# Rocco9999/2048_Q-Learning

Hardware: AMD Instinct MI355X
Metric: env_steps_per_sec (higher is better)
Workload: dtype u8

## Files before the change

### 2048_q-learning_amd/csrc/q2048_kernels.hip

```cpp
#include <hip/hip_runtime.h>
#include <stddef.h>
#include <stdint.h>

#include <cstdio>
#include <cstdlib>
#include <cstring>
#include <ctime>
#include <condition_variable>
#include <deque>
#include <functional>
#include <map>
#include <mutex>
#include <thread>
#include <type_traits>
#include <vector>

#include "q2048_abi.hpp"
#include "q2048_core5.hpp"

#ifdef Q2048_EXPERIMENTS
#define Q2048_XBITS(flags, shift, mask) (((flags) >> (shift)) & (mask))
#else
#define Q2048_XBITS(flags, shift, mask) 0u
#endif
// ... 190 lines not shown
  }
  return kNoSlot;
}

__global__ __launch_bounds__(kBlock) void k_table_summarise(q2048_slot* table, u64 lines) {
  for (u64 l = (u64)blockIdx.x * kBlock + threadIdx.x; l < lines; l += (u64)gridDim.x * kBlock) {
    q2048_slot* s = table + (l << 2);
    u64 sum = 0ull;
#pragma unroll
    for (int r = 0; r < 4; ++r) {
      const u64 k = s[r].key;
      if (k != 0ull) sum |= summary_fp(mix64(k)) << (16 * r);
    }
#pragma unroll
    for (int r = 0; r < 4; ++r) s[r].reserved = sum;
  }
}
__device__ __forceinline__ int64_t probe_find_summary(const q2048_slot* table, u64 mask, const Geo<4>::Key& key,
                                                      Row& row, bool& created, uint32_t maxp = kRolloutProbe) {
  const u64 hash = key_hash(key);
  const Seq sq = seq_of(hash, mask);
  const u64 fp = summary_fp(hash);
  created = false;
  row = Row{0.f, 0.f, 0.f, 0.f};
  for (uint32_t p = 0, lim = probe_limit(mask, maxp); p < lim; p += 4u) {
    const u64 base = ((sq.line0 + (u64)(p >> 2)) & sq.lmask) << 2;
    const u32x4 v = ld16_agent(&table[base | (u64)sq.off].q[2]);
    const u64 sum = (u64)v.z | ((u64)v.w << 32);
    uint32_t e = 0u, m = 0u;
#pragma unroll
    for (uint32_t r = 0; r < 4u; ++r) {
      const u64 f = (sum >> (16u * r)) & 0xffffull;
      e |= (uint32_t)(f == 0ull) << r;
      m |= (uint32_t)(f == fp) << r;
    }
    uint32_t ev = (((e | m) | ((e | m) << 4)) >> sq.off) & 15u;
    while (ev != 0u) {
      const uint32_t j = (uint32_t)__builtin_ctz(ev), r = (sq.off + j) & 3u;
      const u64 i = base | (u64)r;
      if ((e >> r) & 1u) return ~(int64_t)i;
      const u32x4 h = ld16_agent(&table[i]);
      if (((u64)h.x | ((u64)h.y << 32)) == key.k0) {
        u64 hi = (u64)v.x | ((u64)v.y << 32);
        if (j != 0u) hi = ld_u64(&table[i].q[2]);
        row = Row{bits_f32(h.z), bits_f32(h.w), bits_f32((uint32_t)hi), bits_f32((uint32_t)(hi >> 32))};
        return (int64_t)i;
      }
      ev &= ev - 1u;
    }
  }
  return kNoSlot;
}
template <int KEY_WORDS>
__global__ __launch_bounds__(kBlock) void k_table_summarise_side(const q2048_slot* table, u64 lines, u64* side) {
  for (u64 l = (u64)blockIdx.x * kBlock + threadIdx.x; l < lines; l += (u64)gridDim.x * kBlock) {
    const uint4* s = reinterpret_cast<const uint4*>(table + (l << 2));
    u64 sum = 0ull;
#pragma unroll
    for (int r = 0; r < 4; ++r) {
      const uint4 a = s[2 * r];
      const u64 k = (u64)a.x | ((u64)a.y << 32);
      u64 h = k;
      if constexpr (KEY_WORDS == 2) {
        const uint4 b = s[2 * r + 1];
        h = k ^ (((u64)b.z | ((u64)b.w << 32)) * 0x9E3779B97F4A7C15ull);
      }
      if (k != 0ull) sum |= summary_fp(mix64(h)) << (16 * r);
    }
    side[l] = sum;
  }
}
__device__ __forceinline__ int64_t probe_find_summary(const q2048_slot* table, const u64* side, u64 mask,
                                                      const Geo<5>::Key& key, Row& row, bool& created,
                                                      uint32_t maxp = kRolloutProbe) {
  const u64 hash = key_hash(key);
  const Seq sq = seq_of(hash, mask);
  const u64 fp = summary_fp(hash);
  created = false;
  row = Row{0.f, 0.f, 0.f, 0.f};
  for (uint32_t p = 0, lim = probe_limit(mask, maxp); p < lim; p += 4u) {
    const u64 line = (sq.line0 + (u64)(p >> 2)) & sq.lmask;
    SummaryHits hits = summary_decode(ld_u64(&side[line]), fp, sq.off);
    uint32_t r;
    bool absent;
    while (summary_pop(hits, sq.off, r, absent)) {
      const u64 i = (line << 2) | (u64)r;
      if (absent) return ~(int64_t)i;
      const u32x4 a = ld16_agent(&table[i]);
      if (((u64)a.x | ((u64)a.y << 32)) == key.k0) {
        const u32x4 b = ld16_agent(&table[i].q[2]);
        if (((u64)b.z | ((u64)b.w << 32)) == key.k1) {
          row = Row{bits_f32(a.z), bits_f32(a.w), bits_f32(b.x), bits_f32(b.y)};
          return (int64_t)i;
        }
      }
    }
  }
  return kNoSlot;
}
template <bool SUMMARY, class Key>
__device__ __forceinline__ int64_t probe_find_as(const q2048_slot* table, const u64* side, u64 mask, const Key& key,
                                                 Row& row, bool& created) {
  if constexpr (SUMMARY && sizeof(Key) == sizeof(u64)) return probe_find_summary(table, mask, key, row, created);
  else if constexpr (SUMMARY) return probe_find_summary(table, side, mask, key, row, created);
  else return probe_find(table, mask, key, row, created);
}

template <class Key>
__device__ __forceinline__ int64_t probe_insert(q2048_slot* table, u64 mask, const Key& key, u64 start,
                                                bool& inserted, uint32_t maxp = kRolloutProbe) {
  const Seq sq = seq_of(key_hash(key), mask);
  u64 i = start & mask;
  inserted = false;
  u64 k = 0ull;
  for (uint32_t p = seq_pos(sq, i), lim = probe_limit(mask, maxp); p < lim; i = seq_slot(sq, ++p), k = ld_u64(&table[i].key)) {
    if (k == 0ull) k = atomicCAS(reinterpret_cast<u64*>(&table[i].key), 0ull, key.k0);
    if ((k == 0ull || k == key.k0) && confirm(&table[i], key, k == 0ull, inserted)) return (int64_t)i;
  }
  inserted = false;
  return kNoSlot;
}

struct Claim { u64 ret; u64 at; bool active; };

__device__ __forceinline__ int64_t claim_issue(q2048_slot* table, u64, int64_t slot,
                                               const Geo<4>::Key& key, Claim& c, bool&) {
  c.active = slot < 0 && slot != kNoSlot;
  if (c.active) {
    c.at = (u64)~slot;
    c.ret = atomicCAS(reinterpret_cast<u64*>(&table[c.at].key), 0ull, key.k0);
  }
  return slot;
}
__device__ __forceinline__ int64_t claim_issue(q2048_slot* table, u64 mask, int64_t slot,
                                               const Geo<5>::Key& key, Claim& c, bool& inserted) {
  c.active = false;
  if (slot < 0 && slot != kNoSlot) return probe_insert(table, mask, key, (u64)~slot, inserted);
  return slot;
}
template <class Key>
__device__ __forceinline__ int64_t claim_resolve(q2048_slot* table, u64 mask, const Key& key, Claim& c,
                                                 int64_t slot, bool& inserted) {
  if (!c.active) return slot;
  c.active = false;
  if (c.ret == 0ull) { inserted = true; return (int64_t)c.at; }
  if (c.ret == key.k0) return (int64_t)c.at;
  const Seq sq = seq_of(key_hash(key), mask);
  return probe_insert(table, mask, key, seq_slot(sq, seq_pos(sq, c.at) + 1u), inserted);
}

enum : uint32_t { kTdStorePlain = 0, kTdCas = 1, kTdStoreSc1 = 2, kTdStoreNt = 3, kTdNone = 4,
                  kTdAdd = 6 };
struct TdCounters { uint32_t retries, fallbacks; };
__device__ __forceinline__ float td_update(q2048_slot* slot, int a, float guess, float reward,
                                           float max_next, bool done, double lr, double gamma,
                                           TdCounters& ctrs, uint32_t mode, int max_cas = kMaxCas) {
  unsigned int* addr = reinterpret_cast<unsigned int*>(&slot->q[a]);
  unsigned int expect = f32_bits(guess);
  float nq = td_value(guess, reward, max_next, done, lr, gamma);
  if (mode == kTdStorePlain) { *addr = f32_bits(nq); return nq; }
  if (mode == kTdNone) return nq;
#ifdef Q2048_EXPERIMENTS
  if (mode == kTdStoreSc1) {
    __hip_atomic_store(addr, f32_bits(nq), __ATOMIC_RELAXED, __HIP_MEMORY_SCOPE_AGENT);
    return nq;
  }
  if (mode == kTdStoreNt) { __builtin_nontemporal_store(f32_bits(nq), addr); return nq; }
  if (mode == kTdAdd) { atomicAdd(&slot->q[a], nq - guess); return nq; }
#endif
  for (int it = 0; it < max_cas; ++it) {
    const unsigned int prev = atomicCAS(addr, expect, f32_bits(nq));
    if (prev == expect) return nq;
    ++ctrs.retries;
    expect = prev;
    nq = td_value(bits_f32(expect), reward, max_next, done, lr, gamma);
  }
  ++ctrs.fallbacks;
  *addr = f32_bits(nq);
  return nq;
}
__device__ __forceinline__ void flush_pending(q2048_slot* slot, const Row& q, uint32_t& pend) {
  unsigned int* w = reinterpret_cast<unsigned int*>(slot->q);
  if (pend & 1u) w[0] = f32_bits(q.q0);
  if (pend & 2u) w[1] = f32_bits(q.q1);
  if (pend & 4u) w[2] = f32_bits(q.q2);
  if (pend & 8u) w[3] = f32_bits(q.q3);
  pend = 0u;
}
__device__ __forceinline__ uint32_t td_mode_of(uint32_t flags) {
  const uint32_t x = Q2048_XBITS(flags, 8, 15u);
  return x ? x : ((flags & Q2048_FLAG_TD_CAS) ? kTdCas : kTdStorePlain);
}

__device__ __forceinline__ uint32_t wave_count(bool pred) {
  return (uint32_t)__popcll(__ballot(pred));
}
__device__ __forceinline__ bool wave_leader() {
  const u64 active = __ballot(true);
  return (u64)(threadIdx.x & 63) == (u64)__ffsll((long long)active) - 1ull;
}

struct BlockStats {
  u64 i[Q2048_NSTAT_I];
  double f[Q2048_NSTAT_F];
};
__device__ __forceinline__ void stats_clear(BlockStats& s) {
  if (threadIdx.x < Q2048_NSTAT_I) s.i[threadIdx.x] = 0ull;
  if (threadIdx.x < Q2048_NSTAT_F) s.f[threadIdx.x] = 0.0;
  __syncthreads();
}
__device__ __forceinline__ void stats_flush(BlockStats& s, int64_t* gi, double* gf) {
  __syncthreads();
  if (gi != nullptr && threadIdx.x < Q2048_NSTAT_I && s.i[threadIdx.x] != 0ull)
    atomicAdd(reinterpret_cast<u64*>(gi) + threadIdx.x, s.i[threadIdx.x]);
  if (gf != nullptr && threadIdx.x < Q2048_NSTAT_F && s.f[threadIdx.x] != 0.0)
    atomicAdd(gf + threadIdx.x, s.f[threadIdx.x]);
}
constexpr int kStatStripes = 64;
struct StatStripe { u64 i[Q2048_NSTAT_I]; double f[Q2048_NSTAT_F]; };
__device__ __forceinline__ void stats_flush_striped(BlockStats& s, StatStripe* stripes) {
  __syncthreads();
  if (stripes == nullptr) return;
  StatStripe& mine = stripes[blockIdx.x % kStatStripes];
  if (threadIdx.x < Q2048_NSTAT_I && s.i[threadIdx.x] != 0ull) atomicAdd(&mine.i[threadIdx.x], s.i[threadIdx.x]);
  if (threadIdx.x < Q2048_NSTAT_F && s.f[threadIdx.x] != 0.0) atomicAdd(&mine.f[threadIdx.x], s.f[threadIdx.x]);
}
__global__ __launch_bounds__(64) void k_stats_fold(const StatStripe* stripes, int64_t* gi, double* gf) {
  const int t = (int)threadIdx.x;
  if (t < Q2048_NSTAT_I && gi != nullptr) {
    u64 sum = 0ull;
    for (int k = 0; k < kStatStripes; ++k) sum += stripes[k].i[t];
    if (sum) atomicAdd(reinterpret_cast<u64*>(gi) + t, sum);
  } else if (t >= Q2048_NSTAT_I && t < Q2048_NSTAT_I + Q2048_NSTAT_F && gf != nullptr) {
    double sum = 0.0;
    for (int k = 0; k < kStatStripes; ++k) sum += stripes[k].f[t - Q2048_NSTAT_I];
    if (sum != 0.0) atomicAdd(gf + (t - Q2048_NSTAT_I), sum);
  }
}
__device__ __forceinline__ void wait_vm() { asm volatile("s_waitcnt vmcnt(0)" ::: "memory"); }
__device__ __forceinline__ void stats_flush_acked(BlockStats& s, int64_t* gi, double* gf) {
  __syncthreads();
  if (threadIdx.x < Q2048_NSTAT_I && s.i[threadIdx.x] != 0ull) {
    const u64 old = atomicAdd(reinterpret_cast<u64*>(gi) + threadIdx.x, s.i[threadIdx.x]);
    asm volatile("" :: "v"(old));
  }
  if (threadIdx.x < Q2048_NSTAT_F && s.f[threadIdx.x] != 0.0) {
    const double old = atomicAdd(gf + threadIdx.x, s.f[threadIdx.x]);
    asm volatile("" :: "v"(old));
  }
  wait_vm();
}
__device__ __forceinline__ void stats_mirror(const int64_t* gi, const double* gf, u64* mirror, uint32_t* ticket) {
  __shared__ uint32_t my_ticket;
  __syncthreads();
  if (threadIdx.x == 0)
    my_ticket = __hip_atomic_fetch_add(ticket, 1u, __ATOMIC_RELAXED, __HIP_MEMORY_SCOPE_AGENT);
  __syncthreads();
  if (my_ticket != gridDim.x - 1u) return;
  const int t = (int)threadIdx.x;
  if (t < Q2048_NSTAT_I + Q2048_NSTAT_F) {
    const u64* src = t < Q2048_NSTAT_I ? reinterpret_cast<const u64*>(gi) + t
                                       : reinterpret_cast<const u64*>(gf) + (t - Q2048_NSTAT_I);
    const u64 v = __hip_atomic_load(const_cast<u64*>(src), __ATOMIC_RELAXED, __HIP_MEMORY_SCOPE_AGENT);
    __hip_atomic_store(mirror + t, v, __ATOMIC_RELAXED, __HIP_MEMORY_SCOPE_SYSTEM);
  }
  wait_vm();
  __syncthreads();
  if (t == 0) {
    const uint32_t launches = __hip_atomic_load(ticket + 1, __ATOMIC_RELAXED, __HIP_MEMORY_SCOPE_AGENT) + 1u;
    __hip_atomic_store(ticket + 1, launches, __ATOMIC_RELAXED, __HIP_MEMORY_SCOPE_AGENT);
    __hip_atomic_store(mirror + Q2048_MIRROR_SEQ, (u64)launches, __ATOMIC_RELAXED, __HIP_MEMORY_SCOPE_SYSTEM);
    __hip_atomic_store(ticket, 0u, __ATOMIC_RELAXED, __HIP_MEMORY_SCOPE_AGENT);
  }
}
__device__ __forceinline__ void episode_stats(BlockStats& s, const Aux& a, uint32_t max_l2) {
  atomicAdd(&s.i[Q2048_ST_SCORE], (u64)(int64_t)a.score);
  atomicAdd(&s.i[Q2048_ST_HIST0 + (max_l2 > 22u ? 22u : max_l2)], 1ull);
  const double ret = (double)a.ep_return;
  atomicAdd(&s.f[Q2048_SF_RETURN], ret);
  atomicAdd(&s.f[Q2048_SF_RETURN_SQ], ret * ret);
}

template <int N>
__global__ __launch_bounds__(kBlock) void k_env_init(uint8_t* boards, q2048_aux* aux, int64_t B,
                                                     uint64_t seed, uint64_t env_id0) {
  __shared__ Stage<N> st;
  const int64_t i = (int64_t)blockIdx.x * kBlock + threadIdx.x;
  typename Geo<N>::BoardT b;
  Aux a;
  init_env(b, a, seed, env_id0 + (uint64_t)i);
  store_board(boards, i, B, b, st);
  if (i < B) st_aux(aux, i, a);
}

template <int N>
__global__ __launch_bounds__(kBlock) void k_env_reset(uint8_t* boards, q2048_aux* aux,
                                                      const uint8_t* mask, int64_t B, uint64_t seed,
                                                      uint64_t env_id0, uint32_t flags) {
  __shared__ Stage<N> st;
  const int64_t i = (int64_t)blockIdx.x * kBlock + threadIdx.x;
  const bool mine = i < B && (mask == nullptr || mask[i] != 0);
  if constexpr (N == 4) { if (!mine) return; }
  else { if (__ballot(mine) == 0ull) return; }
  auto b = load_board(boards, i, B, st);
  if (mine) {
    Aux a = ld_aux(aux, i);
    begin_episode(b, a, seed, env_id0 + (uint64_t)i, (flags & Q2048_FLAG_RESET_SHAPING) != 0);
    st_aux(aux, i, a);
  }
  store_board(boards, i, B, b, st);
}

template <int N, int ENV>
__global__ __launch_bounds__(kBlock) void k_env_step(const uint8_t* boards_in, uint8_t* boards, q2048_aux* aux,
                                                     const uint8_t* actions, int64_t B, uint64_t seed,
                                                     uint64_t env_id0, uint32_t ctr, float* reward,
                                                     uint8_t* done, uint8_t* max_l2, int32_t* max_tile,
                                                     uint32_t* status,
                                                     const uint32_t* draw_pos, const uint32_t* draw_val,
                                                     const uint32_t* draw_opos, const uint32_t* draw_oval,
                                                     int draw_stride) {
  __shared__ Stage<N> st;
  const int64_t i = (int64_t)blockIdx.x * kBlock + threadIdx.x;
  auto b = load_board(boards_in, i, B, st);
  if (i < B) {
    const int act = actions[i];
    if (act > 3) {
      atomicOr(status, Q2048_STATUS_BAD_ACTION);
// ... 244 lines not shown
  Row r;
  bool made;
  uint32_t g;
  const int64_t slot = probe_find(table, mask, state_key_as<SYM>(b, salt, status, g), r, made, kMaxProbe);
  if constexpr (SYM) r = row_env(r, g);
  reinterpret_cast<float4*>(q_out)[i] = make_float4(r.q0, r.q1, r.q2, r.q3);
  if (found != nullptr) found[i] = slot >= 0;
}

constexpr int kUpdateBlock = 1024;
template <int N, bool FROZEN>
__global__ __launch_bounds__(kUpdateBlock) void k_q_update(q2048_slot* table, u64 mask, const uint8_t* s,
                                                     const uint8_t* actions, const float* reward,
                                                     const uint8_t* s2, const uint8_t* done, int64_t B,
                                                     double lr, double gamma, uint64_t env_id0,
                                                     uint32_t flags, RowCache<N>* cache, int64_t* stats_i,
                                                     uint32_t* status) {
  __shared__ BlockStats bs;
  __shared__ Stage<N, kUpdateBlock / 64> st;
  stats_clear(bs);
  const int64_t i = (int64_t)blockIdx.x * kUpdateBlock + threadIdx.x;
  const auto b_s = load_board(s, i, B, st);
  const auto b_n = load_board(s2, i, B, st);
  if (i < B) {
    const int act = actions[i];
    const float rew = reward[i];
    const bool is_done = done[i] != 0;
    bool ins_n = false, ins_s = false, dropped = false;
    TdCounters tdc{0u, 0u};
    constexpr bool frozen = FROZEN;
    if (act > 3) {
      atomicOr(status, Q2048_STATUS_BAD_ACTION);
    } else {
      const u64 salt = (flags & Q2048_FLAG_INDEPENDENT) ? lane_salt(env_id0 + (uint64_t)i) : 0ull;
      const auto key_s = state_key(b_s, salt, status);
      const auto key_n = state_key(b_n, salt, status);
      const bool same = key_eq(key_n, key_s);
      Row rs;
      int64_t slot = kNoSlot;
      if (cache == nullptr || !cache_get(cache, i, key_s, cache_tag(table, mask), rs, slot, frozen)) {
        slot = probe_find(table, mask, key_s, rs, ins_s);
        if (slot < 0 && slot != kNoSlot && !frozen) slot = probe_insert(table, mask, key_s, (u64)~slot, ins_s);
      }
      Row rn = rs;
      int64_t slot_n = slot;
      Claim claim{0ull, 0ull, false};
      if (!same) {
        slot_n = probe_find(table, mask, key_n, rn, ins_n);
        if constexpr (!frozen) slot_n = claim_issue(table, mask, slot_n, key_n, claim, ins_n);
      }
      const float max_next = max4(rn.q0, rn.q1, rn.q2, rn.q3);
      if (slot >= 0) {
        const float nq = td_update(&table[slot], act, row_get(rs, act), rew, max_next, is_done,
                                   lr, gamma, tdc, td_mode_of(flags));
        if (same) row_set(rn, act, nq);
      } else {
        dropped = true;
        if (!frozen) atomicOr(status, Q2048_STATUS_TABLE_FULL);
        else if (same)
          row_set(rn, act, td_value(row_get(rs, act), rew, max_next, is_done, lr, gamma));
      }
      bool ins_c = false;
      slot_n = claim_resolve(table, mask, key_n, claim, slot_n, ins_c);
      ins_n = ins_n || ins_c;
      if (cache != nullptr) cache_put(cache, i, key_n, cache_tag(table, mask), rn, slot_n, frozen);
    }
    const uint32_t n_ins = wave_count(ins_n) + wave_count(ins_s), n_drop = wave_count(dropped);
    if (tdc.retries) atomicAdd(&bs.i[Q2048_ST_CAS_RETRY], (u64)tdc.retries);
    if (tdc.fallbacks) atomicAdd(&bs.i[Q2048_ST_CAS_FALLBACK], (u64)tdc.fallbacks);
    if (wave_leader()) {
      if (n_ins) atomicAdd(&bs.i[Q2048_ST_INSERTS], (u64)n_ins);
      if (n_drop) atomicAdd(&bs.i[Q2048_ST_DROPS], (u64)n_drop);
    }
  }
  stats_flush(bs, stats_i, nullptr);
}

#ifdef Q2048_FUSED_MIN_WAVES
#define Q2048_FUSED_WAVES(N) Q2048_FUSED_MIN_WAVES
#else
#define Q2048_FUSED_WAVES(N) ((N) == 4 ? 6 : 5)
#endif
constexpr int kModeLearn = 0, kModeCas = 1, kModeEval = 2, kModeFrozen = 4, kModeSummary = 8;
constexpr int kModeSym = 16;
constexpr int kFusedBlockBig = 512, kFusedBlockSmall = kBlock;
constexpr int64_t kFusedBigBatch = 786432;
#ifdef Q2048_EXPERIMENTS
__device__ unsigned long long* g_timeline;
#define Q2048_STAMP(k) do { if (g_timeline != nullptr && threadIdx.x == 0) {                       \
    g_timeline[(size_t)blockIdx.x * 8 + (k)] = wall_clock64();                                     \
    if ((k) == 0) {                                                                                \
      g_timeline[(size_t)blockIdx.x * 8 + 4] = (unsigned)__builtin_amdgcn_s_getreg((31 << 11) | 4);   \
      g_timeline[(size_t)blockIdx.x * 8 + 5] = (unsigned)__builtin_amdgcn_s_getreg((31 << 11) | 20);  \
    } } } while (0)
#else
#define Q2048_STAMP(k) do { } while (0)
#endif
__device__ const LutImage g_lut_image = Q2048_LUT_IMAGE;
template <int N, int ENV, int MODE, int BLOCK>
__global__ __launch_bounds__(BLOCK, Q2048_FUSED_WAVES(N)) void k_fused_rollout(
    uint8_t* boards, q2048_aux* aux, q2048_slot* table, u64 mask, int64_t B, int steps, double eps,
    double lr, double gamma, uint64_t seed, uint64_t env_id0, uint32_t ctr0, uint32_t flags,
    int64_t* stats_i, double* stats_f, uint32_t* status, q2048_episode* log, int64_t log_cap,
    u64* log_count, void* row_cache, u64* mirror, uint32_t* ticket, const u64* side) {
  RowCache<N>* const cache = static_cast<RowCache<N>*>(row_cache);
  __shared__ BlockStats bs;
  __shared__ Stage<N, BLOCK / 64> st;
  __shared__ LutImage lut_lds;
  static_assert(BLOCK >= kLutImageDoubles, "one double of the image per thread");
  Q2048_STAMP(0);
  if (threadIdx.x < kLutImageDoubles)
    reinterpret_cast<double*>(&lut_lds)[threadIdx.x] = reinterpret_cast<const double*>(&g_lut_image)[threadIdx.x];
  stats_clear(bs);
  const ImageLuts lut{&lut_lds};
  const int64_t i = (int64_t)blockIdx.x * BLOCK + threadIdx.x;
  auto b = load_board(boards, i, B, st);
  if (i < B) {
    const uint64_t id = env_id0 + (uint64_t)i;
    const u64 salt = (flags & Q2048_FLAG_INDEPENDENT) ? lane_salt(id) : 0ull;
    constexpr bool play_only = (ENV & kEnvPlayOnly) != 0;
    constexpr bool no_learn = (MODE & ~kModeSym) == kModeEval;
    constexpr bool sym = (MODE & kModeSym) != 0;
    static_assert(!sym || (N == 4 && !play_only), "symmetry folding: 4x4 learners, evaluators and frozen tables");
    constexpr bool frozen = (MODE & kModeFrozen) != 0;
    constexpr bool summary = (MODE & kModeSummary) != 0;
#ifdef Q2048_EXPERIMENTS
    const uint32_t td_mode = no_learn ? (uint32_t)kTdNone : td_mode_of(flags);
    const bool x_noclaim = ((flags >> 12) & 1u) || play_only || no_learn || frozen, x_noprobe = ((flags >> 13) & 1u) || play_only;
    const bool may_defer = td_mode == kTdStorePlain && !((flags >> 14) & 1u);
    const int max_cas = ((flags >> 16) & 0xffu) ? (int)((flags >> 16) & 0xffu) : kMaxCas;
#else
    constexpr uint32_t td_mode = no_learn ? kTdNone : ((MODE & kModeCas) ? kTdCas : kTdStorePlain);
    constexpr bool x_noclaim = play_only || no_learn || frozen, x_noprobe = play_only;
    constexpr bool may_defer = td_mode == kTdStorePlain;
    constexpr int max_cas = kMaxCas;
#endif
    Aux a = ld_aux(aux, i);
    uint32_t g_s;
    auto key_s = state_key_as<sym>(b, salt, status, g_s);
    Row q{0.f, 0.f, 0.f, 0.f};
    bool made0 = false;
    int64_t slot_s = kNoSlot;
    if (!play_only && (cache == nullptr || !cache_get(cache, i, key_s, cache_tag(table, mask), q, slot_s, frozen)))
      slot_s = probe_find_as<summary>(table, side, mask, key_s, q, made0);
    Claim claim{0ull, 0ull, false};
    uint32_t n_valid = 0, n_explore = 0, n_done = 0, n_insert = wave_count(made0), n_drop = 0;
    uint32_t pend = 0;
    TdCounters tdc{0u, 0u};
    double reward_sum = 0.0;
    const DrawPrep prep_x = draws_prepare(seed, id, kStreamStep);
    const uint64_t eps_t = eps_threshold(eps);

    for (int t = 0; t < steps; ++t) {
      const Draws x = draws_at(prep_x, ctr0 + (uint32_t)t);
      Draws y{0u, 0u, 0u, 0u};
      if constexpr ((ENV & kEnvDqn) != 0) y = draws(seed, id, ctr0 + (uint32_t)t, kStreamOver);
      bool explored;
      Row qe = q;
      if constexpr (sym) qe = row_env(q, g_s);
      const int act_env = eps_greedy_at(eps_t, x.x0, x.x1, qe.q0, qe.q1, qe.q2, qe.q3, explored);
      const StepOut o = env_step_profile<ENV>(b, a, act_env, x.x2, x.x3, y.x0, y.x1, lut);
      const int act = sym ? sym_action(g_s, act_env) : act_env;
      uint32_t g_n;
      const auto key_n = state_key_as<sym>(b, salt, status, g_n);
      const bool same = key_eq(key_n, key_s);
      bool ins_s = false, ins_n = false;
      slot_s = claim_resolve(table, mask, key_s, claim, slot_s, ins_s);
      if (slot_s < 0 && slot_s != kNoSlot && !x_noclaim)
        slot_s = probe_insert(table, mask, key_s, (u64)~slot_s, ins_s);
      Row qn = q;
      int64_t slot_n = slot_s;
      if (!same) {
        if (x_noprobe) { qn = Row{0.f, 0.f, 0.f, 0.f}; slot_n = ~(int64_t)key_home(key_n, mask); }
        else slot_n = probe_find_as<summary>(table, side, mask, key_n, qn, ins_n);
      }
      const float max_next = max4(qn.q0, qn.q1, qn.q2, qn.q3);
      float nq = 0.f;
      const bool updated = slot_s >= 0;
      if (updated) {
        if (same && !o.done && may_defer) {
          nq = td_value(row_get(q, act), o.reward, max_next, false, lr, gamma);
          pend |= 1u << act;
        } else {
          nq = td_update(&table[slot_s], act, row_get(q, act), o.reward, max_next, o.done != 0, lr,
                         gamma, tdc, td_mode, max_cas);
          pend &= ~(1u << act);
          if (pend) flush_pending(&table[slot_s], q, pend);
        }
      } else if (frozen) {
        nq = td_value(row_get(q, act), o.reward, max_next, o.done != 0, lr, gamma);
      }
      if (o.done) {
        if (!same && slot_n < 0 && slot_n != kNoSlot && !x_noclaim)
          probe_insert(table, mask, key_n, (u64)~slot_n, ins_n);
        episode_stats(bs, a, o.max_log2);
        if (log != nullptr) {
          const u64 at = atomicAdd(log_count, 1ull);
          if ((int64_t)at < log_cap) {
            Row ql = q;
            if ((updated || frozen) && !no_learn) row_set(ql, act, nq);
            if constexpr (sym) ql = row_env(ql, g_s);
            q2048_episode rec;
            rec.env_id = id; rec.episode = a.episode; rec.action = (uint8_t)act_env;
            rec.max_log2 = o.max_log2; rec.steps_lo = (uint16_t)(ctr0 + (uint32_t)t);
            rec.reward = o.reward; rec.total_return = a.ep_return; rec.score = a.score;
            rec.q[0] = ql.q0; rec.q[1] = ql.q1; rec.q[2] = ql.q2; rec.q[3] = ql.q3;
            rec.reserved = 0u;
            log[at] = rec;
          }
        }
        begin_episode(b, a, seed, id, (ENV & kEnvResetShaping) != 0);
        key_s = state_key_as<sym>(b, salt, status, g_s);
        bool made = false;
        q = Row{0.f, 0.f, 0.f, 0.f};
        slot_s = play_only ? kNoSlot : probe_find_as<summary>(table, side, mask, key_s, q, made);
        ins_n = ins_n || made;
      } else if (same) {
        if ((updated || frozen) && !no_learn) row_set(q, act, nq);
        else if (!updated) slot_s = kNoSlot;
      } else {
        key_s = key_n; slot_s = slot_n; q = qn; g_s = g_n;
        if (!x_noclaim) {
          bool made = false;
          slot_s = claim_issue(table, mask, slot_s, key_s, claim, made);
          ins_n = ins_n || made;
        }
      }
      n_valid += wave_count(o.valid != 0);
      n_explore += wave_count(explored);
      n_insert += wave_count(ins_s) + wave_count(ins_n);
      n_drop += wave_count(!updated && !play_only && !no_learn);
      n_done += wave_count(o.done != 0);
      reward_sum += (double)o.reward;
      if (t == 0) Q2048_STAMP(1);
    }
    Q2048_STAMP(2);
    if (pend && slot_s >= 0) flush_pending(&table[slot_s], q, pend);
    bool ins_last = false;
    slot_s = claim_resolve(table, mask, key_s, claim, slot_s, ins_last);
    n_insert += wave_count(ins_last);
    st_aux(aux, i, a);
    if (!play_only && cache != nullptr) cache_put(cache, i, key_s, cache_tag(table, mask), q, slot_s, frozen);

    if (n_drop && !frozen) atomicOr(status, Q2048_STATUS_TABLE_FULL);
    if (tdc.retries) atomicAdd(&bs.i[Q2048_ST_CAS_RETRY], (u64)tdc.retries);
    if (tdc.fallbacks) atomicAdd(&bs.i[Q2048_ST_CAS_FALLBACK], (u64)tdc.fallbacks);
    atomicAdd(&bs.f[Q2048_SF_REWARD], reward_sum);
    const uint32_t n_active = wave_count(true);
    if (wave_leader()) {
      atomicAdd(&bs.i[Q2048_ST_STEPS], (u64)n_active * (u64)steps);
      atomicAdd(&bs.i[Q2048_ST_VALID], (u64)n_valid);
      atomicAdd(&bs.i[Q2048_ST_EXPLORE], (u64)n_explore);
      atomicAdd(&bs.i[Q2048_ST_EPISODES], (u64)n_done);
      atomicAdd(&bs.i[Q2048_ST_INSERTS], (u64)n_insert);
      atomicAdd(&bs.i[Q2048_ST_DROPS], (u64)n_drop);
    }
  }
  store_board(boards, i, B, b, st);
  if (mirror == nullptr) {
    stats_flush(bs, stats_i, stats_f);
  } else {
    stats_flush_acked(bs, stats_i, stats_f);
    stats_mirror(stats_i, stats_f, mirror, ticket);
  }
  Q2048_STAMP(3);
}

template <int N, int ENV, bool SYM = false>
__global__ __launch_bounds__(kBlock) void k_play_rollout(
    uint8_t* boards, q2048_aux* aux, const q2048_slot* table, u64 mask, int64_t B, int steps, double eps,
    uint64_t seed, uint64_t env_id0, uint32_t ctr0, uint32_t flags, int64_t* stats_i, double* stats_f,
    uint32_t* status) {
  __shared__ BlockStats bs;
  __shared__ Stage<N> st;
  __shared__ LutImage lut_lds;
  static_assert(kBlock >= kLutImageDoubles, "one double of the image per thread");
  if (threadIdx.x < kLutImageDoubles)
    reinterpret_cast<double*>(&lut_lds)[threadIdx.x] = reinterpret_cast<const double*>(&g_lut_image)[threadIdx.x];
  stats_clear(bs);
  const ImageLuts lut{&lut_lds};
  const int64_t i = (int64_t)blockIdx.x * kBlock + threadIdx.x;
  auto b = load_board(boards, i, B, st);
  if (i < B) {
    const uint64_t id = env_id0 + (uint64_t)i;
    const u64 salt = (flags & Q2048_FLAG_INDEPENDENT) ? lane_salt(id) : 0ull;
    Aux a = ld_aux(aux, i);
    uint32_t n_valid = 0, n_explore = 0, n_done = 0;
    double reward_sum = 0.0;
    const DrawPrep prep_x = draws_prepare(seed, id, kStreamStep);
    const uint64_t eps_t = eps_threshold(eps);
    for (int t = 0; t < steps; ++t) {
      const Draws x = draws_at(prep_x, ctr0 + (uint32_t)t);
      Draws y{0u, 0u, 0u, 0u};
      if constexpr ((ENV & kEnvDqn) != 0) y = draws(seed, id, ctr0 + (uint32_t)t, kStreamOver);
      Row q;
      bool made;
      uint32_t g;
      probe_find(table, mask, state_key_as<SYM>(b, salt, status, g), q, made, kMaxProbe);
      if constexpr (SYM) q = row_env(q, g);
      bool explored;
      const int act = play_action(legal_mask(b), q.q0, q.q1, q.q2, q.q3, eps_t, x.x0, x.x1, explored);
      const StepOut o = env_step_profile<ENV>(b, a, act, x.x2, x.x3, y.x0, y.x1, lut);
      if (o.done) {
        episode_stats(bs, a, o.max_log2);
        begin_episode(b, a, seed, id, (ENV & kEnvResetShaping) != 0);
      }
      n_valid += wave_count(o.valid != 0);
      n_explore += wave_count(explored);
      n_done += wave_count(o.done != 0);
      reward_sum += (double)o.reward;
    }
    st_aux(aux, i, a);
    atomicAdd(&bs.f[Q2048_SF_REWARD], reward_sum);
    const uint32_t n_active = wave_count(true);
    if (wave_leader()) {
      atomicAdd(&bs.i[Q2048_ST_STEPS], (u64)n_active * (u64)steps);
      atomicAdd(&bs.i[Q2048_ST_VALID], (u64)n_valid);
      atomicAdd(&bs.i[Q2048_ST_EXPLORE], (u64)n_explore);
      atomicAdd(&bs.i[Q2048_ST_EPISODES], (u64)n_done);
    }
  }
  store_board(boards, i, B, b, st);
  stats_flush(bs, stats_i, stats_f);
}

constexpr int kDetHashShift = 44, kDetHashBits = 16;
constexpr u64 kDetSlotMask = (1ull << kDetHashShift) - 1ull;
constexpr u64 kDetDrop = 1ull << 62, kDetDone = 1ull << 63;
constexpr uint32_t kNoCarry = 0xffffffffu;
__device__ __forceinline__ Row ld_row(const q2048_slot* s) {
  const u32x4 v = ld16_agent(&s->q[0]);
  return Row{bits_f32(v.x), bits_f32(v.y), bits_f32(v.z), bits_f32(v.w)};
}
template <int N, int ENV, bool VISITS>
__device__ __forceinline__ void det_phase1_body(
    uint8_t* boards, q2048_aux* aux, q2048_slot* table, u64 mask, int64_t B, double eps, double gamma,
    uint64_t seed, uint64_t env_id0, uint32_t ctr, uint32_t flags, u64* group_out, double* target_out,
    uint32_t* carry, int use_carry, StatStripe* stat_stripes, uint32_t* gs0, int n_gs, uint32_t* status,
    RowCache<N>* cache, double lr) {
  __shared__ BlockStats bs;
  __shared__ Stage<N> st;
  stats_clear(bs);
  const int64_t i = (int64_t)blockIdx.x * kBlock + threadIdx.x;
  for (int64_t idx = i; idx < (int64_t)n_gs; idx += (int64_t)gridDim.x * kBlock) gs0[idx] = 0u;
  auto b = load_board(boards, i, B, st);
  if (i < B) {
    const uint64_t id = env_id0 + (uint64_t)i;
    const u64 salt = (flags & Q2048_FLAG_INDEPENDENT) ? lane_salt(id) : 0ull;
    Aux a = ld_aux(aux, i);
    const auto key_s = state_key(b, salt, status);
    const u64 hash_s = key_hash(key_s);
    const Draws x = draws(seed, id, ctr, kStreamStep);
    Draws y{0u, 0u, 0u, 0u};
    if constexpr ((ENV & kEnvDqn) != 0) y = draws(seed, id, ctr, kStreamOver);
    Row q{0.f, 0.f, 0.f, 0.f}, qn;
    bool ins_s = false, ins_n = false, dropped = false;
    const bool frozen = (flags & Q2048_FLAG_NO_NEW_ROWS) != 0u;
    const uint32_t held = use_carry ? carry[i] : kNoCarry;
    constexpr bool visits = VISITS;
    int64_t slot_s;
    if (held != kNoCarry) {
      slot_s = (int64_t)held;
      if (!(draw_uniform(x.x0) < eps)) q = ld_row(&table[slot_s]);
    } else {
      slot_s = probe_find(table, mask, key_s, q, ins_s);
      if (slot_s < 0 && slot_s != kNoSlot && !frozen) slot_s = probe_insert(table, mask, key_s, (u64)~slot_s, ins_s);
      if (slot_s < 0) { dropped = true; if (!frozen || slot_s == kNoSlot) atomicOr(status, Q2048_STATUS_TABLE_FULL); }
      if constexpr (visits) {
        if (slot_s < 0) {
          Row v;
          int64_t at;
          if (cache_get(cache, i, key_s, cache_tag(table, mask), v, at, true) && at == kNoSlot) q = v;
        }
      }
    }
    bool explored;
    const int act = eps_greedy(eps, x.x0, x.x1, q.q0, q.q1, q.q2, q.q3, explored);
    const StepOut o = env_step_profile<ENV>(b, a, act, x.x2, x.x3, y.x0, y.x1);
// ... 3656 lines not shown
```

Baseline: 22.59 billion.

## Skip next-state probe on terminal steps and defer missed-slot inserts via claims

On terminal transitions the TD update now uses a specialized terminal value that ignores max_next, so the next-state probe is skipped and only the fresh episode's start state is probed. Missing-key inserts that used to be synchronous probe_insert calls are now issued as asynchronous claims, at the top of the next iteration or on the terminal path, and resolved later. This aims to cut hash-table probes and serialized atomic inserts per step. It restructures the claim/resolve ordering and the terminal bookkeeping, which risks subtle changes in insert counts or in which slot gets updated.

```diff
diff --git a/2048_q-learning_amd/csrc/q2048_kernels.hip b/2048_q-learning_amd/csrc/q2048_kernels.hip
--- a/2048_q-learning_amd/csrc/q2048_kernels.hip
+++ b/2048_q-learning_amd/csrc/q2048_kernels.hip
@@ -366,12 +366,21 @@
 enum : uint32_t { kTdStorePlain = 0, kTdCas = 1, kTdStoreSc1 = 2, kTdStoreNt = 3, kTdNone = 4,
                   kTdAdd = 6 };
 struct TdCounters { uint32_t retries, fallbacks; };
+__device__ __forceinline__ float td_value_terminal(float q_sa, float reward, double lr) {
+  Q2048_NO_CONTRACT
+  return (float)td_fold((double)q_sa, (double)reward + 0.0, lr);
+}
+template <bool TERMINAL = false>
 __device__ __forceinline__ float td_update(q2048_slot* slot, int a, float guess, float reward,
                                            float max_next, bool done, double lr, double gamma,
                                            TdCounters& ctrs, uint32_t mode, int max_cas = kMaxCas) {
+  const auto value = [&](float q_sa) {
+    if constexpr (TERMINAL) return td_value_terminal(q_sa, reward, lr);
+    else return td_value(q_sa, reward, max_next, done, lr, gamma);
+  };
   unsigned int* addr = reinterpret_cast<unsigned int*>(&slot->q[a]);
   unsigned int expect = f32_bits(guess);
-  float nq = td_value(guess, reward, max_next, done, lr, gamma);
+  float nq = value(guess);
   if (mode == kTdStorePlain) { *addr = f32_bits(nq); return nq; }
   if (mode == kTdNone) return nq;
 #ifdef Q2048_EXPERIMENTS
@@ -387,7 +396,7 @@
     if (prev == expect) return nq;
     ++ctrs.retries;
     expect = prev;
-    nq = td_value(bits_f32(expect), reward, max_next, done, lr, gamma);
+    nq = value(bits_f32(expect));
   }
   ++ctrs.fallbacks;
   *addr = f32_bits(nq);
@@ -938,6 +947,9 @@
     const uint64_t eps_t = eps_threshold(eps);
 
     for (int t = 0; t < steps; ++t) {
+      bool ins_s = false, ins_n = false;
+      if (!x_noclaim && !claim.active && slot_s < 0 && slot_s != kNoSlot)
+        slot_s = claim_issue(table, mask, slot_s, key_s, claim, ins_s);
       const Draws x = draws_at(prep_x, ctr0 + (uint32_t)t);
       Draws y{0u, 0u, 0u, 0u};
       if constexpr ((ENV & kEnvDqn) != 0) y = draws(seed, id, ctr0 + (uint32_t)t, kStreamOver);
@@ -948,37 +960,29 @@
       const StepOut o = env_step_profile<ENV>(b, a, act_env, x.x2, x.x3, y.x0, y.x1, lut);
       const int act = sym ? sym_action(g_s, act_env) : act_env;
       uint32_t g_n;
-      const auto key_n = state_key_as<sym>(b, salt, status, g_n);
+      auto key_n = state_key_as<sym>(b, salt, status, g_n);
       const bool same = key_eq(key_n, key_s);
-      bool ins_s = false, ins_n = false;
-      slot_s = claim_resolve(table, mask, key_s, claim, slot_s, ins_s);
-      if (slot_s < 0 && slot_s != kNoSlot && !x_noclaim)
-        slot_s = probe_insert(table, mask, key_s, (u64)~slot_s, ins_s);
-      Row qn = q;
-      int64_t slot_n = slot_s;
-      if (!same) {
-        if (x_noprobe) { qn = Row{0.f, 0.f, 0.f, 0.f}; slot_n = ~(int64_t)key_home(key_n, mask); }
-        else slot_n = probe_find_as<summary>(table, side, mask, key_n, qn, ins_n);
+      {
+        bool ins_c = false;
+        slot_s = claim_resolve(table, mask, key_s, claim, slot_s, ins_c);
+        ins_s = ins_s || ins_c;
       }
-      const float max_next = max4(qn.q0, qn.q1, qn.q2, qn.q3);
+      const bool updated = slot_s >= 0;
       float nq = 0.f;
-      const bool updated = slot_s >= 0;
-      if (updated) {
-        if (same && !o.done && may_defer) {
-          nq = td_value(row_get(q, act), o.reward, max_next, false, lr, gamma);
-          pend |= 1u << act;
-        } else {
-          nq = td_update(&table[slot_s], act, row_get(q, act), o.reward, max_next, o.done != 0, lr,
-                         gamma, tdc, td_mode, max_cas);
+      if (o.done) {
+        if (updated) {
+          nq = td_update<true>(&table[slot_s], act, row_get(q, act), o.reward, 0.f, true, lr, gamma, tdc, td_mode, max_cas);
           pend &= ~(1u << act);
           if (pend) flush_pending(&table[slot_s], q, pend);
+        } else if (frozen) {
+          nq = td_value_terminal(row_get(q, act), o.reward, lr);
         }
-      } else if (frozen) {
-        nq = td_value(row_get(q, act), o.reward, max_next, o.done != 0, lr, gamma);
-      }
-      if (o.done) {
-        if (!same && slot_n < 0 && slot_n != kNoSlot && !x_noclaim)
-          probe_insert(table, mask, key_n, (u64)~slot_n, ins_n);
+        if (!same && !x_noclaim) {
+          bool made = false;
+          claim_issue(table, mask, ~(int64_t)key_home(key_n, mask), key_n, claim, made);
+          ins_n = made;
+          key_s = key_n;
+        }
         episode_stats(bs, a, o.max_log2);
         if (log != nullptr) {
           const u64 at = atomicAdd(log_count, 1ull);
@@ -996,20 +1000,50 @@
           }
         }
         begin_episode(b, a, seed, id, (ENV & kEnvResetShaping) != 0);
-        key_s = state_key_as<sym>(b, salt, status, g_s);
+        key_n = state_key_as<sym>(b, salt, status, g_n);
+      }
+      Row qn = q;
+      int64_t slot_n = slot_s;
+      if (o.done ? !play_only : (!same && !x_noprobe)) {
         bool made = false;
-        q = Row{0.f, 0.f, 0.f, 0.f};
-        slot_s = play_only ? kNoSlot : probe_find_as<summary>(table, side, mask, key_s, q, made);
+        slot_n = probe_find_as<summary>(table, side, mask, key_n, qn, made);
+      } else if (o.done) {
+        qn = Row{0.f, 0.f, 0.f, 0.f};
+        slot_n = kNoSlot;
+      } else if (!same) {
+        qn = Row{0.f, 0.f, 0.f, 0.f};
+        slot_n = ~(int64_t)key_home(key_n, mask);
+      }
+      if (o.done) {
+        bool made = false;
+        claim_resolve(table, mask, key_s, claim, kNoSlot, made);
         ins_n = ins_n || made;
-      } else if (same) {
-        if ((updated || frozen) && !no_learn) row_set(q, act, nq);
-        else if (!updated) slot_s = kNoSlot;
+        key_s = key_n; slot_s = slot_n; q = qn; g_s = g_n;
       } else {
-        key_s = key_n; slot_s = slot_n; q = qn; g_s = g_n;
-        if (!x_noclaim) {
-          bool made = false;
-          slot_s = claim_issue(table, mask, slot_s, key_s, claim, made);
-          ins_n = ins_n || made;
+        const float max_next = max4(qn.q0, qn.q1, qn.q2, qn.q3);
+        if (updated) {
+          if (same && may_defer) {
+            nq = td_value(row_get(q, act), o.reward, max_next, false, lr, gamma);
+            pend |= 1u << act;
+          } else {
+            nq = td_update(&table[slot_s], act, row_get(q, act), o.reward, max_next, false, lr, gamma, tdc, td_mode,
+                           max_cas);
+            pend &= ~(1u << act);
+            if (pend) flush_pending(&table[slot_s], q, pend);
+          }
+        } else if (frozen) {
+          nq = td_value(row_get(q, act), o.reward, max_next, false, lr, gamma);
+        }
+        if (same) {
+          if ((updated || frozen) && !no_learn) row_set(q, act, nq);
+          else if (!updated) slot_s = kNoSlot;
+        } else {
+          key_s = key_n; slot_s = slot_n; q = qn; g_s = g_n;
+          if (!x_noclaim) {
+            bool made = false;
+            slot_s = claim_issue(table, mask, slot_s, key_s, claim, made);
+            ins_n = ins_n || made;
+          }
         }
       }
       n_valid += wave_count(o.valid != 0);
```

Result: slower. 22.29 billion (-1.4%).
